# tkob-vh/umi-collapse-rs

Measured on AMD Instinct MI355X. Metric: UMI-pair Hamming comparisons/s, effective (W pairs of the positions / hot-path time; 12-bp UMIs, all-pairs adjacency + directional collapse; the n-gram partition compares walked_fraction of W, the all-pairs kernels' result bit for bit), higher is better.
Workload: dtype u32; 1 GPU; BASELINE config 2 per GPU: 1000000 reads, 12-bp UMIs, one alignment position (uniform UMIs), --data naive --algo dir -k 1 -p 0.5; standard=True, reads_per_rank=1000000, positions_per_rank=1, unique_umis_rank0=970714, pairs_W_total=471142349541, parallelism=one GPU

## Files before the change

umi_collapse_rs_amd/csrc/umihip_internal.h:

```cpp
#pragma once

#include <hip/hip_runtime_api.h>
#include <stdint.h>

namespace umihip {

struct PairTask {
    uint32_t row0;
    uint32_t row_end;
    uint32_t col0;
    uint32_t col1;
};

enum PairMode : int {
    MODE_DIRECTIONAL = 0,
    MODE_ADJACENCY = 1,
    MODE_NEIGHBOURS = 2,
    MODE_CLUSTER = 3,
};

enum Counter : int {
    CNT_EDGES = 0,
    CNT_CANDIDATES = 1,
    CNT_ERROR = 2,
// ... 157 lines not shown
    uint32_t *bin_start;
    unsigned long long *scan_state;
    SegTask *tasks;
    uint32_t task_cap;
    void *sub_rec;
    const RangeTask *ranges;
    uint32_t n_ranges;
    const SegBlock *blocks;
    uint32_t n_blocks;
    uint32_t lds_bins;
    uint32_t parts_per_pass;
    uint2 *priv_edges;
    uint8_t *priv_dist;
    uint32_t *priv_cnt;
    uint2 *priv_stat;
    uint32_t *uf_parent;
    const uint64_t *prep_keys, *prep_nmask;
    const int32_t *prep_freq;
    int32_t *prep_thr;
    uint32_t *prep_label;
    uint32_t *prep_lab;
    float prep_percentage;
    unsigned long long *prep_counters;
    int umi_len;
    int key_words;
    int full_umi_len;
    uint32_t use_ckey;
    uint32_t col_sliced;
    uint32_t local_cap;
    uint32_t probe_rest, probe_min;
    uint32_t super_cap;
    const SegSuper *supers;
    uint32_t n_supers;
};
hipError_t launch_seg_build(const SegArgs &g, void *fkey, const int32_t *freq, bool key32,
                            unsigned long long *counters, hipStream_t s);
constexpr uint32_t SEG_PRIV_CAP = 512;
int seg_pair_blocks_per_cu(bool key32, bool has_n, bool ckey);
hipError_t launch_seg_pairs(const PairArgs &a, const SegArgs &g, bool key32, float percentage,
                            uint32_t part, uint32_t n_parts, uint32_t n_blocks, hipStream_t s);
hipError_t launch_seg_edge_append(const PairArgs &a, const SegArgs &g, uint32_t n_blocks, hipStream_t s);
constexpr uint32_t SEG_LOCAL_MAX_CAP = 2048;
constexpr uint32_t SEG_LOCAL_CAP = 512;
constexpr int SEG_PROBE_MAX_REST = 6;
constexpr uint32_t SEG_PROBE_WORDS = (1u << (2 * SEG_PROBE_MAX_REST)) / 32;
constexpr uint32_t SEG_PROBE_MIN = 129;
constexpr int SEG_SUPER_MAX_REST = 8;
constexpr uint32_t SEG_SUPER_WORDS = (1u << (2 * SEG_SUPER_MAX_REST)) / 32;
constexpr int SEG_SUPER_MAX_BASES = 4;
constexpr uint32_t SEG_SUPER_MAX_CAP = 8192;
constexpr uint32_t SEG_SUPER_CAP = 5632;
constexpr uint32_t SEG_SUPER_MIN = 1024;
constexpr uint32_t SEG_SUPER_SMALL = 2048;
inline uint32_t seg_super_threads(uint32_t cap) { return cap <= SEG_SUPER_SMALL ? 256u : 1024u; }
size_t seg_super_lds_bytes(uint32_t cap);
uint32_t seg_super_blocks(uint32_t n_supers, uint32_t n_cus);
hipError_t launch_seg_super(const PairArgs &a, const SegArgs &g, float percentage, uint32_t n_blocks, hipStream_t s);
size_t seg_local_lds_bytes(uint32_t cap);
int seg_local_blocks_per_cu(bool has_n, uint32_t cap);
hipError_t launch_seg_local(const PairArgs &a, const SegArgs &g, float percentage, uint32_t n_blocks, hipStream_t s);

hipError_t launch_wide_pairs(const PairArgs &a, uint32_t n_tasks, int n_words, hipStream_t s);

hipError_t launch_edit_prep(const uint64_t *keys, const uint64_t *nmask, const int32_t *freq, const uint64_t *bucket_off,
                            uint64_t n_buckets, uint32_t n, int umi_len, float percentage, uint64_t *planes,
                            uint32_t *counts, int32_t *thr, uint32_t *label, unsigned long long *counters, hipStream_t s);
hipError_t launch_edit_pairs(const PairArgs &a, const uint32_t *counts, uint32_t n_tasks, int umi_len, hipStream_t s);
// ... 252 lines not shown
```

umi_collapse_rs_amd/csrc/umihip_pipeline.cpp:

```cpp
#include "umihip_host.hpp"

#include <algorithm>
#include <chrono>

using namespace umihip;

namespace {

template <class LaunchRound>
int run_rounds(umi_ctx *ctx, hipStream_t s, LaunchRound launch_round, int &rounds, int batch = 4)
{
    uint32_t *d_changed = ctx->d_changed();
    for (;;) {
        HIP_TRY(hipMemsetAsync(d_changed, 0, sizeof(uint32_t) * MAX_ROUNDS_PER_SYNC, s));
        for (int r = 0; r < batch; r++) HIP_TRY(launch_round(d_changed, r));
        HIP_TRY(hipMemcpyAsync(ctx->h_changed(), d_changed, sizeof(uint32_t) * batch, hipMemcpyDeviceToHost, s));
        HIP_TRY(hipStreamSynchronize(s));
        bool done = false;
        for (int r = 0; r < batch && !done; r++) {
            rounds++;
            done = ctx->h_changed()[r] == 0;
        }
        if (done) return UMI_OK;
        if (rounds > MAX_ROUNDS) return fail(UMI_ERR_HIP, "label propagation diverged");
// ... 257 lines not shown
            if ((rc = ctx->status.reserve(n)) || (rc = ctx->blocked.reserve(n))) return rc;
        if (edit && (rc = ctx->planes.reserve((size_t)n * 4))) return rc;
        d_cnt = ctx->counters.as<unsigned long long>();
        bs_fkey = ctx->fkey.p;
        return UMI_OK;
    }

    void plan_host()
    {
        scan_table_range(bucket_off, 0, n_buckets, fused_max, nullptr, ctx->table_pass);
        const bool dev_tiles = mode != MODE_CLUSTER;
        const bool seg_on = ctx->seg_index && need_pairs && !(ctx->prune && dev_tiles) && !edit;
        SegSuperOpt sup;
        sup.on = ctx->seg_super && ctx->seg_unite && ctx->seg_ckey && unions_collapse() && n_parts == 1 && ctx->two_phase == 2 &&
                 key32 && !wide() && !edit && !d_nmask;
        sup.bases = ctx->seg_super_bases;
        sup.cap = ctx->seg_super_cap;
        sup.min = ctx->seg_super_min;
        build_plan(bucket_off, n_buckets, wide() || edit ? 0x7FFFFFFFu : ctx->small_max,
                   ctx->use_bitslice && k <= BS_MAX_K && !wide() && !edit && dev_tiles,
                   plan_umi_len(), fused_max, ctx->prune && dev_tiles, ctx->bs_sorted && ctx->bs_unit == 2 && need_pairs && dev_tiles,
                   ctx->bs_tables && key32 && dev_tiles, ctx->bs_tab_min_run, seg_on ? std::max(ctx->seg_min, 1u) : 0u, k, key32, pl,
                   &ctx->table_pass, sup);
        prune = ctx->prune && dev_tiles && need_pairs && !pl.bs_buckets.empty() && !wide() && !edit;
        keep_my_share(pl.small_tasks);
        keep_my_share(pl.big_tasks);
        st.max_bucket = pl.max_bucket;
        st.n_pairs = pl.n_pairs;
    }

    size_t seg_bins_bytes() const { return (pl.seg_bins * 4 + 15) & ~(size_t)15; }
    size_t seg_zero_bytes() const
    {
        return (seg_bins_bytes() + (1 + pl.seg_chunks.size()) * sizeof(unsigned long long) + 15) & ~(size_t)15;
    }

    int upload_plan()
    {
        int rc;
        size_t off = 0;
        auto place = [&](size_t bytes) {
            const size_t at = off;
            off = (off + bytes + 63) & ~(size_t)63;
            return at;
        };
        const size_t o_ranges = place(pl.ranges.size() * sizeof(RangeTask));
        const size_t o_segs = place(pl.segs.size() * sizeof(SegDesc));
        const size_t o_chunks = place(pl.seg_chunks.size() * sizeof(SegScanChunk));
        const size_t o_blocks = place(pl.seg_blocks.size() * sizeof(SegBlock));
        const size_t o_supers = place(pl.seg_supers.size() * sizeof(SegSuper));
        const size_t o_small = place(pl.small_tasks.size() * sizeof(PairTask));
        const size_t o_big = place(pl.big_tasks.size() * sizeof(PairTask));
        const size_t total = std::max<size_t>(off, 64);
        PinnedBuf &hp = ctx->h_plan_alt[ctx->plan_flip];
        if ((rc = hp.reserve(total)) || (rc = ctx->plan_tables.reserve(total))) return rc;
        if (off) memset(hp.p, 0, off);
        if ((rc = hp.put(o_ranges, pl.ranges.data(), pl.ranges.size() * sizeof(RangeTask))) ||
            (rc = hp.put(o_segs, pl.segs.data(), pl.segs.size() * sizeof(SegDesc))) ||
            (rc = hp.put(o_chunks, pl.seg_chunks.data(), pl.seg_chunks.size() * sizeof(SegScanChunk))) ||
            (rc = hp.put(o_blocks, pl.seg_blocks.data(), pl.seg_blocks.size() * sizeof(SegBlock))) ||
            (rc = hp.put(o_supers, pl.seg_supers.data(), pl.seg_supers.size() * sizeof(SegSuper))) ||
            (rc = hp.put(o_small, pl.small_tasks.data(), pl.small_tasks.size() * sizeof(PairTask))) ||
            (rc = hp.put(o_big, pl.big_tasks.data(), pl.big_tasks.size() * sizeof(PairTask))))
            return rc;
        const PinnedBuf &prev = ctx->h_plan_alt[ctx->plan_flip ^ 1];
        const bool same = off && ctx->plan_uploaded == off && ctx->plan_uploaded_to == ctx->plan_tables.p &&
                          prev.p && prev.cap >= off && memcmp(prev.p, hp.p, off) == 0;
// ... 400 lines not shown
        const PairArgs a = pair_args(ovf_cap);
        if (pl.seg_parts) {
            const uint32_t blocks = std::max(1u, (uint32_t)std::min<uint64_t>(
                pl.seg_task_cap, ctx->seg_blocks ? ctx->seg_blocks : (uint64_t)ctx->n_cus * std::min(16u, seg_occupancy())));
            const uint32_t local_blocks = seg.local_cap && seg_local_bins ? (uint32_t)std::max<uint64_t>(1, std::min<uint64_t>(
                                                              seg_local_bins, (uint64_t)ctx->n_cus * seg_local_occupancy()))
                                                        : 0u;
            const uint32_t super_blocks = seg.super_cap ? seg_super_blocks(seg.n_supers, (uint32_t)ctx->n_cus) : 0u;
            const uint32_t super_slots = super_blocks * (seg_super_threads(seg.super_cap) / 64u);
            const size_t slots = (size_t)local_blocks + super_slots + blocks;
            if ((rc = ctx->seg_priv_edges.reserve(slots * SEG_PRIV_CAP * sizeof(uint2))) ||
                (rc = ctx->seg_priv_cnt.reserve(slots * 4)) || (rc = ctx->seg_priv_stat.reserve(slots * sizeof(uint2))) ||
                (mode == MODE_NEIGHBOURS && (rc = ctx->seg_priv_dist.reserve((size_t)blocks * SEG_PRIV_CAP))))
                return rc;
            seg.priv_edges = ctx->seg_priv_edges.as<uint2>();
            seg.priv_dist = ctx->seg_priv_dist.as<uint8_t>();
            seg.priv_cnt = ctx->seg_priv_cnt.as<uint32_t>();
            seg.uf_parent = one_sync() && ctx->seg_unite ? ctx->label.as<uint32_t>() : nullptr;
            const bool slots_to_collapse = seg.uf_parent && unions_collapse();
            seg.priv_stat = slots_to_collapse ? ctx->seg_priv_stat.as<uint2>() : nullptr;
            if ((seg.local_cap || seg.super_cap) && !seg.uf_parent)
                return fail(UMI_ERR_HIP, "internal: part-0 sub-buckets planned for the local kernel without unions");
            SegArgs super_seg = seg;
            super_seg.priv_edges += (size_t)local_blocks * SEG_PRIV_CAP;
            super_seg.priv_cnt += local_blocks;
            if (super_seg.priv_stat) super_seg.priv_stat += local_blocks;
            SegArgs pair_seg = super_seg;
            pair_seg.priv_edges += (size_t)super_slots * SEG_PRIV_CAP;
            pair_seg.priv_cnt += super_slots;
            if (pair_seg.priv_stat) pair_seg.priv_stat += super_slots;

            if (prof) HIP_TRY(hipEventRecord(ctx->ev[7], s));
            if (local_blocks) HIP_TRY(launch_seg_local(a, seg, percentage, local_blocks, s));
            if (super_blocks) HIP_TRY(launch_seg_super(a, super_seg, percentage, super_blocks, s));
            HIP_TRY(launch_seg_pairs(a, pair_seg, key32, percentage, part, n_parts, blocks, s));
            if (prof) HIP_TRY(hipEventRecord(ctx->ev[8], s));
            seg_timed = true;
            priv_blocks_for_collapse = slots_to_collapse ? (uint32_t)slots : 0u;
            if (!priv_blocks_for_collapse) HIP_TRY(launch_seg_edge_append(a, seg, blocks, s));
            st.n_pair_launches += 1;
        }
        if ((rc = enqueue_legacy_tiles(a))) return rc;
        if (edit) {
            if (prof) HIP_TRY(hipEventRecord(ctx->ev[7], s));
            HIP_TRY(launch_edit_pairs(a, ctx->planes.as<uint32_t>(), (uint32_t)pl.small_tasks.size(), umi_len, s));
            if (prof) HIP_TRY(hipEventRecord(ctx->ev[8], s));
            edit_timed = true;
            st.n_pair_launches += pl.small_tasks.empty() ? 0 : 1;
            return UMI_OK;
        }
        if (wide()) {
            HIP_TRY(launch_wide_pairs(a, (uint32_t)pl.small_tasks.size(), n_words, s));
            st.n_pair_launches += pl.small_tasks.empty() ? 0 : 1;
            return UMI_OK;
        }
        PairArgs big = a;
        big.tasks = d_big;
        HIP_TRY(launch_pairs(big, (uint32_t)pl.big_tasks.size(), true, key32, s));
        HIP_TRY(launch_pairs(a, (uint32_t)pl.small_tasks.size(), false, key32, s));
        for (auto &v : pl.bs_tasks) st.n_pair_launches += v.empty() ? 0 : 1;
        st.n_pair_launches += pl.tab_rows.empty() ? 0 : 2;
        st.n_pair_launches += (pl.small_tasks.empty() ? 0 : 1) + (pl.big_tasks.empty() ? 0 : 1);
        return UMI_OK;
    }

    int note_pair_counters()
    {
// ... 387 lines not shown
```

umi_collapse_rs_amd/csrc/umihip_seg.hip:

```cpp
#include <hip/hip_runtime.h>

#include "umihip_internal.h"
#include "umihip_device.h"

namespace umihip {

namespace {

constexpr int SCAN_THREADS = 256;
constexpr int SCAN_PER_THREAD = SEG_SCAN_CHUNK / SCAN_THREADS;

__device__ __forceinline__ bool probe_part(const SegArgs &g, uint32_t nb)
{
    return g.probe_rest != 0u && g.umi_len - (int)nb <= (int)g.probe_rest;
}
__device__ __forceinline__ bool local_bin(const SegArgs &g, uint32_t part, uint32_t c) { return part == 0 && c <= g.local_cap; }
__device__ __forceinline__ bool super_taken(const SegArgs &g, uint32_t n) { return n >= 2u && n <= g.super_cap; }
__device__ __forceinline__ uint32_t super_bases(const SegArgs &g, uint32_t seg) { return g.super_cap ? g.segs[seg].sup_g : 0u; }

constexpr unsigned long long SCAN_HAVE = 1ull << 63, SCAN_PREFIX = 1ull << 31;
__device__ __forceinline__ unsigned long long scan_pack(uint32_t e, uint32_t t) { return ((unsigned long long)e << 32) | t; }
__global__ __launch_bounds__(SCAN_THREADS) void seg_scan_kernel(SegArgs g, unsigned long long *counters)
{
    __shared__ uint2 wsum[SCAN_THREADS / 64];
    __shared__ uint32_t my_chunk;
    __shared__ uint2 prefix;
    unsigned long long *ticket = g.scan_state, *status = g.scan_state + 1;
    if (threadIdx.x == 0) my_chunk = (uint32_t)atomicAdd(ticket, 1ull);
    __syncthreads();
    const uint32_t ci = my_chunk;
    const SegScanChunk ch = g.chunks[ci];
    uint32_t c[SCAN_PER_THREAD];
    uint2 mine = make_uint2(0u, 0u);
    const uint32_t b_first = threadIdx.x * SCAN_PER_THREAD;
#pragma unroll
    for (int q = 0; q < SCAN_PER_THREAD; q++) {
        const uint32_t b = b_first + q;
        c[q] = b < ch.nbins ? g.bin_cnt[ch.bin0 + b] : 0u;
        mine.x += c[q];
    }
    uint32_t no_tasks = 0;
    const uint32_t sg = ch.part == 0 ? super_bases(g, ch.seg) : 0u;
    if (sg) {
        static_assert(SCAN_PER_THREAD == 1 || SCAN_PER_THREAD == 4, "a super-bin is whole threads' bins");
        __shared__ uint32_t tcnt[SCAN_THREADS];
        tcnt[threadIdx.x] = mine.x;
        __syncthreads();
        const uint32_t nthr = (1u << (2 * sg)) / SCAN_PER_THREAD, t0 = threadIdx.x & ~(nthr - 1u);
        uint32_t n_super = 0;
        for (uint32_t i = 0; i < nthr; i++) n_super += tcnt[t0 + i];
        if (super_taken(g, n_super)) no_tasks = (1u << SCAN_PER_THREAD) - 1u;
    } else {
#pragma unroll
        for (int q = 0; q < SCAN_PER_THREAD; q++)
            if (local_bin(g, ch.part, c[q])) no_tasks |= 1u << q;
    }
#pragma unroll
    for (int q = 0; q < SCAN_PER_THREAD; q++) mine.y += (no_tasks >> q) & 1u ? 0u : seg_tasks_of_bin(c[q]);
    uint2 incl = mine;
    for (int d = 1; d < 64; d <<= 1) {
        const uint32_t ux = __shfl_up(incl.x, d), uy = __shfl_up(incl.y, d);
        if ((int)(threadIdx.x & 63) >= d) {
            incl.x += ux;
            incl.y += uy;
        }
    }
    if ((threadIdx.x & 63) == 63) wsum[threadIdx.x >> 6] = incl;
    __syncthreads();
    if (threadIdx.x < 64) {
        uint2 tot = make_uint2(0u, 0u);
        for (int w = 0; w < SCAN_THREADS / 64; w++) {
            tot.x += wsum[w].x;
            tot.y += wsum[w].y;
        }
        const int lane = threadIdx.x;
        if (lane == 0)
            __hip_atomic_store(&status[ci], SCAN_HAVE | (ci == 0 ? SCAN_PREFIX : 0ull) | scan_pack(tot.x, tot.y),
                               __ATOMIC_RELEASE, __HIP_MEMORY_SCOPE_AGENT);
        uint2 before = make_uint2(0u, 0u);
        int64_t j0 = (int64_t)ci - 1;
        while (j0 >= 0) {
            const int64_t j = j0 - lane;
            unsigned long long st = SCAN_HAVE | SCAN_PREFIX;
            if (j >= 0)
// ... 323 lines not shown
            "v_addc_co_u32_e64 %0, vcc, %0, %0, %11\n\t"
            "v_addc_co_u32_e64 %0, vcc, %0, %0, %12"
            : "+v"(h), "=&s"(s0), "=&s"(s1), "=&s"(s2), "=&s"(s3), "=&v"(t0), "=&v"(t1), "=&v"(t2), "=&v"(t3),
              "=&s"(p0), "=&s"(p1), "=&s"(p2), "=&s"(p3)
            : "v"(x), "v"(ky), "s"(lim2), "n"(J), "n"(J - 1), "n"(J - 2), "n"(J - 3)
            : "vcc");
        return h;
    }
#pragma unroll
    for (int j = J; j > J - 4; j--) h = h + h + (within_k(x ^ readlane_key(ky, j), k) ? 1u : 0u);
    return h;
}
template <bool CK, int J> __device__ __forceinline__ uint32_t four_columns(uint32_t h, uint64_t x, uint64_t ky, int k, uint32_t)
{
#pragma unroll
    for (int j = J; j > J - 4; j--) h = h + h + (within_k(x ^ readlane_key(ky, j), k) ? 1u : 0u);
    return h;
}
template <bool CK, int BASE, typename KeyT>
__device__ __forceinline__ uint32_t columns32(KeyT x, KeyT ky, int k, uint32_t lim2)
{
    uint32_t h = 0;
    h = four_columns<CK, BASE + 31>(h, x, ky, k, lim2);
    h = four_columns<CK, BASE + 27>(h, x, ky, k, lim2);
    h = four_columns<CK, BASE + 23>(h, x, ky, k, lim2);
    h = four_columns<CK, BASE + 19>(h, x, ky, k, lim2);
    h = four_columns<CK, BASE + 15>(h, x, ky, k, lim2);
    h = four_columns<CK, BASE + 11>(h, x, ky, k, lim2);
    h = four_columns<CK, BASE + 7>(h, x, ky, k, lim2);
    h = four_columns<CK, BASE + 3>(h, x, ky, k, lim2);
    return h;
}

template <int K, int NB> __device__ __forceinline__ unsigned long long columns64_sliced(uint32_t x, uint32_t ky)
{
    uint32_t cl[K + 1], ch[K + 1];
#pragma unroll
    for (int l = 0; l <= K; l++) cl[l] = ch[l] = 0u;
#pragma unroll
    for (int b = 0; b < NB; b++) {
        const unsigned long long p0 = __ballot((ky & (1u << (3 * b))) != 0u), p1 = __ballot((ky & (2u << (3 * b))) != 0u);
        const uint32_t r0 = (uint32_t)((int32_t)(x << (31 - 3 * b)) >> 31), r1 = (uint32_t)((int32_t)(x << (30 - 3 * b)) >> 31);
        const uint32_t dl = BITOP3((uint32_t)p0 ^ r0, (uint32_t)p1, r1, TT_A | (TT_B ^ TT_C));
        const uint32_t dh = BITOP3((uint32_t)(p0 >> 32) ^ r0, (uint32_t)(p1 >> 32), r1, TT_A | (TT_B ^ TT_C));
#pragma unroll
        for (int l = K; l >= 1; l--) {
            cl[l] = BITOP3(cl[l], cl[l - 1], dl, TT_A | (TT_B & TT_C));
            ch[l] = BITOP3(ch[l], ch[l - 1], dh, TT_A | (TT_B & TT_C));
        }
        cl[0] |= dl;
        ch[0] |= dh;
    }
    return ~(((unsigned long long)ch[K] << 32) | cl[K]);
}
template <int K> __device__ __forceinline__ unsigned long long columns64_sliced_nb(uint32_t x, uint32_t ky, int nb)
{
    switch (nb) {
    case 1: return columns64_sliced<K, 1>(x, ky);
    case 2: return columns64_sliced<K, 2>(x, ky);
    case 3: return columns64_sliced<K, 3>(x, ky);
    case 4: return columns64_sliced<K, 4>(x, ky);
    case 5: return columns64_sliced<K, 5>(x, ky);
    case 6: return columns64_sliced<K, 6>(x, ky);
    case 7: return columns64_sliced<K, 7>(x, ky);
    case 8: return columns64_sliced<K, 8>(x, ky);
    case 9: return columns64_sliced<K, 9>(x, ky);
    default: return columns64_sliced<K, 10>(x, ky);
    }
}
__device__ __forceinline__ unsigned long long columns64_sliced_k(uint32_t x, uint32_t ky, int k, int nb)
{
    switch (k) {
    case 0: return columns64_sliced_nb<0>(x, ky, nb);
    case 1: return columns64_sliced_nb<1>(x, ky, nb);
    case 2: return columns64_sliced_nb<2>(x, ky, nb);
    default: return columns64_sliced_nb<3>(x, ky, nb);
    }
}
__device__ __forceinline__ unsigned long long columns64_sliced_k(uint64_t, uint64_t, int, int) { return 0ull; }

template <int ILP>
__device__ __forceinline__ void uf_union_multi(uint32_t *parent, uint32_t (&u)[ILP], uint32_t (&v)[ILP], bool (&act)[ILP])
{
    uint32_t pu[ILP], pv[ILP];
    uint32_t seen[ILP];
#pragma unroll
    for (int s = 0; s < ILP; s++) seen[s] = act[s] ? atomicCAS(&parent[v[s]], v[s], u[s]) : 0u;
#pragma unroll
    for (int s = 0; s < ILP; s++) act[s] = act[s] && seen[s] != v[s] && seen[s] != u[s];
#pragma unroll
    for (int s = 0; s < ILP; s++) {
        pu[s] = act[s] ? ld_parent(&parent[u[s]]) : 0u;
        pv[s] = seen[s];
    }
    for (;;) {
        bool cas[ILP], any = false;
#pragma unroll
        for (int s = 0; s < ILP; s++) {
            act[s] = act[s] && pu[s] != pv[s];
            if (act[s] && pu[s] < pv[s]) {
                uint32_t t = u[s]; u[s] = v[s]; v[s] = t;
                t = pu[s]; pu[s] = pv[s]; pv[s] = t;
            }
            cas[s] = act[s] && u[s] == pu[s];
            any = any || act[s];
        }
        if (!any) break;
        uint32_t r[ILP];
#pragma unroll
        for (int s = 0; s < ILP; s++)
            r[s] = !act[s] ? 0u : cas[s] ? atomicCAS(&parent[u[s]], u[s], pv[s]) : ld_parent(&parent[pu[s]]);
#pragma unroll
// ... 7 lines not shown
                pu[s] = r[s];
            }
        }
    }
}

template <typename KeyT, bool HAS_N, bool CK, int W = 1>
__global__ __launch_bounds__(64) void seg_pair_kernel(PairArgs a, SegArgs g, float percentage,
                                                      uint32_t part, uint32_t n_parts)
{
    using Rec = typename SegRecOf<KeyT>::type;
    constexpr int ILP = 1;
    constexpr uint32_t DRAIN_AT = 64 * ILP;
    constexpr uint32_t HITQ = DRAIN_AT + 64;
    __shared__ EdgeStage stage;
    __shared__ uint2 hitq[HITQ];
    const int lane = threadIdx.x;
    const Rec *__restrict__ sub = (const Rec *)g.sub_rec;
    const uint4 *__restrict__ task_words = (const uint4 *)g.tasks;
    const bool with_dist = a.mode == MODE_NEIGHBOURS;
    if (lane == 0) {
        stage.count = 0;
        stage.candidates = 0;
    }
    __syncthreads();
    const uint32_t n_tasks = (uint32_t)min((unsigned long long)g.task_cap, a.counters[CNT_SEG_TASKS]);
    unsigned int n_cand = 0, n_direct = 0;
    const uint32_t lim2 = (uint32_t)__builtin_amdgcn_readfirstlane(2 * a.k);
    KeyT dup_mask[SEG_MAX_PARTS - 1];
#pragma unroll
    for (int j = 0; j < SEG_MAX_PARTS - 1; j++) dup_mask[j] = KeyT(0);
    uint32_t have_seg = SEG_NONE, have_part = 0;
    int ck_bases = 0;
    uint32_t sup_mask = 0, sup_bins = 0, sup_bin0 = 0;
    const bool sliced = a.k <= 3 && g.col_sliced != 0;
    uint32_t nq = 0;

    auto drain = [&]() {
        __builtin_amdgcn_wave_barrier();
        for (uint32_t q0 = 0; q0 < nq; q0 += 64 * ILP) {
            Rec ra[ILP], cb[ILP];
            bool live[ILP];
#pragma unroll
            for (int s = 0; s < ILP; s++) {
                const uint32_t q = q0 + (uint32_t)s * 64u + (uint32_t)lane;
                live[s] = q < nq;
                const uint2 h = live[s] ? hitq[q] : make_uint2(0u, 0u);
                ra[s] = sub[live[s] ? h.x : 0u];
                cb[s] = sub[live[s] ? h.y : 0u];
            }
            uint32_t uu[ILP], uv[ILP];
            bool unite[ILP];
#pragma unroll
            for (int s = 0; s < ILP; s++) {
                unite[s] = false;
                uu[s] = uv[s] = 0;
                if (!live[s]) continue;
                const KeyT z = ra[s].key ^ cb[s].key;
                bool ok = true;
#pragma unroll
                for (int p = 0; p < SEG_MAX_PARTS - 1; p++)
                    ok = ok && (dup_mask[p] == KeyT(0) || (z & dup_mask[p]) != KeyT(0));
                if (!ok) continue;
                if (sup_bins && ((uint32_t)z & sup_mask) == 0u) {
                    const uint32_t b = sup_bin0 + ((uint32_t)ra[s].key & sup_mask);
                    if (super_taken(g, g.bin_start[b + sup_bins] - g.bin_start[b])) continue;
                }
// ... 72 lines not shown
    uint4 tw = t < n_tasks ? task_words[t] : none;
    uint4 tw1 = t + stride < n_tasks && t + stride > t ? task_words[t + stride] : none;
    KeyT x, ky;
    task_keys(tw, t < n_tasks, x, ky);
    while (t < n_tasks) {
        const uint32_t t1 = t + stride, t2 = t1 + stride;
        const bool has1 = t1 < n_tasks && t1 > t, has2 = has1 && t2 < n_tasks && t2 > t1;
        const uint4 tw2 = has2 ? task_words[t2] : none;
        KeyT x1, ky1;
        task_keys(tw1, has1, x1, ky1);
        const uint32_t row0 = __builtin_amdgcn_readfirstlane(tw.x);
        const uint32_t end = __builtin_amdgcn_readfirstlane(tw.y);
        const uint32_t col0 = __builtin_amdgcn_readfirstlane(tw.z);
        const uint32_t where = __builtin_amdgcn_readfirstlane(tw.w);
        const uint32_t seg = where & 0xFFFFFFu, my_part = (where >> 24) & 15u;
        const uint32_t col1 = (uint32_t)min((unsigned long long)end, (unsigned long long)col0 + (64ull << (where >> 28)));
        const bool mine = !(n_parts > 1 && (((end ^ (end >> 7)) * 0x9E3779B1u) >> 8) % n_parts != part);
        if (mine) {
            const uint32_t n_rows = min(64u, end - row0);
            const uint32_t r = row0 + (uint32_t)lane;
            if (seg != have_seg || my_part != have_part) {
                if (nq) drain();
                const SegDesc *__restrict__ sd = g.segs + seg;
#pragma unroll
                for (int j = 0; j < SEG_MAX_PARTS - 1; j++)
                    dup_mask[j] = (uint32_t)j < my_part ? (KeyT)sd->mask[j] : KeyT(0);
                have_seg = seg;
                have_part = my_part;
                ck_bases = __builtin_amdgcn_readfirstlane(g.umi_len - (int)sd->nb[my_part]);
                const uint32_t sg = my_part != 0 ? super_bases(g, seg) : 0u;
                sup_mask = sg ? ((1u << (2 * (sd->nb[0] - sg))) - 1u) << (2 * sg) : 0u;
                sup_bins = sg ? 1u << (2 * sg) : 0u;
                sup_bin0 = sd->bin_off[0];
            }
            for (uint32_t c0 = col0; c0 < col1; c0 += 64) {
                const uint32_t cn_pos = c0 + 64u + (uint32_t)lane;
                KeyT kn = pad_col<KeyT>();
                if (c0 + 64u < col1 && cn_pos < end) kn = loop_key<CK>(sub[cn_pos]);
                const uint32_t nc = min(64u, end - c0);
                unsigned long long h;
                if (CK && sliced) {
                    h = columns64_sliced_k(x, ky, a.k, ck_bases);
                } else {
                    uint32_t hlo = 0, hhi = 0;
                    hlo = columns32<CK, 0>(x, ky, a.k, lim2);
                    if (nc > 32) hhi = columns32<CK, 32>(x, ky, a.k, lim2);
                    h = ((unsigned long long)hhi << 32) | hlo;
                }
                const int j_min = lane + 1 - (int)(c0 - row0);
                if (nc < 64) h &= (1ull << nc) - 1ull;
                if (j_min > 0) h = j_min >= 64 ? 0ull : h & ~((1ull << j_min) - 1ull);
                if ((uint32_t)lane >= n_rows) h = 0ull;
                while (__any(h != 0ull)) {
                    const unsigned long long bal = __ballot(h != 0ull);
                    if (h) {
                        const int j = __builtin_ctzll(h);
                        h &= h - 1ull;
                        hitq[nq + (uint32_t)__builtin_popcountll(bal & ((1ull << lane) - 1ull))] =
                            make_uint2(r, c0 + (uint32_t)j);
                    }
                    nq += (uint32_t)__builtin_popcountll(bal);
                    if (nq >= DRAIN_AT) drain();
                }
                ky = kn;
            }
        }
        if (!has1) break;
        t = t1;
        tw = tw1;
        tw1 = tw2;
        x = x1;
        ky = ky1;
    }
    if (nq) drain();
    {
// ... 257 lines not shown
                            h &= h - 1ull;
                            hit = r | ((c0 + (uint32_t)j) << 16);
                        }
                        push(has, hit);
                    }
                }
            }
        }
        if (nq) drain();
        for (uint32_t p = lane; p < c; p += 64) {
            uint32_t q = lds_ld(&par[p]);
            for (;;) {
                const uint32_t up = lds_ld(&par[q]);
                if (up == q) break;
                q = up;
            }
            ck[p] = q;
            fr[p] = 0xFFFFFFFFu;
        }
        __syncthreads();
        for (uint32_t p = lane; p < c; p += 64) atomicMin(&fr[ck[p]], ix[p]);
        __syncthreads();
        for (uint32_t p = lane; p < c; p += 64) g.uf_parent[ix[p]] = fr[ck[p]];
        __syncthreads();
    }
    if (lane == 0) g.priv_cnt[blockIdx.x] = min(n_out, SEG_PRIV_CAP);
    for (int off = 32; off > 0; off >>= 1) n_cand += __shfl_down(n_cand, off);
    for (int off = 32; off > 0; off >>= 1) n_direct += __shfl_down(n_direct, off);
    if (lane == 0) g.priv_stat[blockIdx.x] = make_uint2(n_cand, n_direct);
}

constexpr int SUPER_RPT = 8;

template <bool CLUSTER, int NT>
__global__ __launch_bounds__(NT) void seg_super_kernel(PairArgs a, SegArgs g, float percentage)
{
    extern __shared__ uint32_t lds[];
    constexpr int NW = NT / 64;
    constexpr int WPT = (int)SEG_SUPER_WORDS / NT;
    static_assert(WPT * NT == (int)SEG_SUPER_WORDS && WPT >= 1, "whole words per thread");
    const uint32_t cap = g.super_cap;
    uint32_t *sc = lds, *ix = lds + cap, *fr = lds + 2 * cap, *par = lds + 3 * cap;
    uint32_t *bm = lds + 4 * cap, *pre = bm + SEG_SUPER_WORDS;
    __shared__ uint32_t wsum[NW];
    const uint32_t tid = threadIdx.x, wave = tid >> 6;
    const int lane = (int)(tid & 63u);
    const SegRec32 *__restrict__ sub = (const SegRec32 *)g.sub_rec;
    unsigned int n_cand = 0, n_direct = 0;
    const size_t my_slot = (size_t)blockIdx.x * NW + wave;
    uint32_t n_out = 0;
    uint2 *__restrict__ slot = g.priv_edges + my_slot * SEG_PRIV_CAP;
    auto emit = [&](bool has, uint32_t u, uint32_t v) {
        const unsigned long long bal = __ballot(has);
        if (!bal) return;
        const uint32_t cnt = (uint32_t)__builtin_popcountll(bal);
        const uint32_t pos = n_out + (uint32_t)__builtin_popcountll(bal & ((1ull << lane) - 1ull));
        unsigned long long base = 0;
        if (n_out + cnt > SEG_PRIV_CAP) {
            const uint32_t first_over = max(n_out, SEG_PRIV_CAP);
            const int leader = __builtin_ctzll(bal);
            if (lane == leader) base = atomicAdd(&a.counters[CNT_EDGES], (unsigned long long)(n_out + cnt - first_over));
            base = __shfl(base, leader);
            base -= first_over;
        }
        if (has) {
            if (pos < SEG_PRIV_CAP) slot[pos] = make_uint2(u, v);
            else if (base + pos < a.edge_cap) a.edges[base + pos] = make_uint2(u, v);
        }
        n_out += cnt;
    };
    auto decide = [&](bool has, uint32_t pa, uint32_t pb) {
        const uint32_t ia = ix[pa], ib = ix[pb];
        const int32_t fa = (int32_t)fr[pa], fb = (int32_t)fr[pb];
        const bool sw = ib < ia;
        const uint32_t gi = sw ? ib : ia, gj = sw ? ia : ib;
        const int32_t fi = sw ? fb : fa, fj = sw ? fa : fb;
        if (has) n_cand++;
        const bool fwd = has && (CLUSTER || fj <= threshold_of(percentage, fi));
        const bool bwd = has && (CLUSTER || fi <= threshold_of(percentage, fj));
        if (fwd && bwd) {
            n_direct++;
            lds_union_halving(par, min(pa, pb), max(pa, pb));
        }
        emit(fwd != bwd, fwd ? gi : gj, fwd ? gj : gi);
    };

    for (uint32_t u = blockIdx.x; u < g.n_supers; u += gridDim.x) {
        const SegSuper su = g.supers[u];
        const uint32_t start = __builtin_amdgcn_readfirstlane(g.bin_start[su.bin0]);
        const uint32_t c = __builtin_amdgcn_readfirstlane(g.bin_start[su.bin0 + (1u << (2 * su.g))]) - start;
        if (!super_taken(g, c)) continue;
        const uint32_t lo_bits = 2u * su.g, hi_shift = 2u * su.nb, rest = su.rest;
        const uint32_t lo_mask = (1u << lo_bits) - 1u, code_mask = (1u << (2u * rest)) - 1u;
        for (uint32_t w = tid; w < SEG_SUPER_WORDS; w += NT) bm[w] = 0u;
        uint32_t rc[SUPER_RPT], ri[SUPER_RPT], rf[SUPER_RPT], rq[SUPER_RPT];
#pragma unroll
        for (int r = 0; r < SUPER_RPT; r++) {
            const uint32_t p = tid + (uint32_t)r * NT;
            rc[r] = ri[r] = rf[r] = rq[r] = 0u;
            if (p < c) {
                const SegRec32 rec = sub[start + p];
                rc[r] = ((rec.key & lo_mask) | ((rec.key >> hi_shift) << lo_bits)) & code_mask;
                ri[r] = rec.idx;
                rf[r] = (uint32_t)rec.freq;
            }
        }
        __syncthreads();
        bool twice = false;
#pragma unroll
        for (int r = 0; r < SUPER_RPT; r++)
            if (tid + (uint32_t)r * NT < c) {
                const uint32_t bit = 1u << (rc[r] & 31u);
                twice = twice || (atomicOr(&bm[rc[r] >> 5], bit) & bit) != 0u;
            }
        const bool dup = __syncthreads_or(twice ? 1 : 0) != 0;
        if (!dup) {
            {
                uint32_t n_w[WPT], mine = 0;
#pragma unroll
                for (int i = 0; i < WPT; i++) mine += n_w[i] = (uint32_t)__builtin_popcount(bm[tid * WPT + i]);
                uint32_t incl = mine;
                for (int d = 1; d < 64; d <<= 1) {
                    const uint32_t up = __shfl_up(incl, d);
                    if (lane >= d) incl += up;
                }
                if (lane == 63) wsum[wave] = incl;
                __syncthreads();
                uint32_t before = incl - mine;
                for (uint32_t w = 0; w < wave; w++) before += wsum[w];
#pragma unroll
                for (int i = 0; i < WPT; i++) {
                    pre[tid * WPT + i] = before;
                    before += n_w[i];
                }
            }
            __syncthreads();
            auto rank_of = [&](uint32_t s) {
                return pre[s >> 5] + (uint32_t)__builtin_popcount(bm[s >> 5] & ((1u << (s & 31u)) - 1u));
            };
#pragma unroll
            for (int r = 0; r < SUPER_RPT; r++)
                if (tid + (uint32_t)r * NT < c) {
                    const uint32_t q = rank_of(rc[r]);
                    rq[r] = q;
                    sc[q] = rc[r];
                    ix[q] = ri[r];
                    fr[q] = rf[r];
                    par[q] = q;
                }
            __syncthreads();
#pragma unroll
            for (int r = 0; r < SUPER_RPT; r++) {
                if ((uint32_t)r * NT >= c) break;
                const uint32_t s = rc[r];
                uint32_t m = 0;
#pragma unroll
                for (int bb = 0; bb < SEG_SUPER_MAX_REST; bb++) {
#pragma unroll
                    for (int d = 1; d <= 3; d++) {
                        const uint32_t t = s ^ ((uint32_t)d << (2 * bb));
                        const uint32_t there = (bm[t >> 5] >> (t & 31u)) & 1u;
                        if ((uint32_t)bb < rest && t > s) m |= there << (3 * bb + d - 1);
                    }
                }
                if (tid + (uint32_t)r * NT >= c) m = 0u;
                while (__any(m != 0u)) {
                    const bool has = m != 0u;
                    uint32_t pb = 0;
                    if (has) {
                        const int j = __builtin_ctz(m), bb = j / 3;
                        m &= m - 1u;
                        pb = rank_of(s ^ ((uint32_t)(j - 3 * bb + 1) << (2 * bb)));
                    }
                    decide(has, has ? rq[r] : 0u, pb);
                }
            }
        } else {
#pragma unroll
            for (int r = 0; r < SUPER_RPT; r++) {
                const uint32_t p = tid + (uint32_t)r * NT;
                if (p < c) {
                    sc[p] = rc[r];
                    ix[p] = ri[r];
                    fr[p] = rf[r];
                    par[p] = p;
                }
            }
            __syncthreads();
#pragma unroll
            for (int r = 0; r < SUPER_RPT; r++) {
                if ((uint32_t)r * NT >= c) break;
                const uint32_t p = tid + (uint32_t)r * NT, p_first = p - (uint32_t)lane;
                const uint32_t s = rc[r];
                const uint32_t n_it = c > p_first + 1u ? c - 1u - p_first : 0u;
                for (uint32_t i = 1; i <= n_it; i++) {
                    const uint32_t q = p + i;
                    const uint32_t z = s ^ (q < c ? sc[q] : 0u);
                    const bool hit = p < c && q < c && __builtin_popcount((z | (z >> 1)) & 0x55555555u) <= 1;
                    if (__any(hit)) decide(hit, hit ? p : 0u, hit ? q : 0u);
                }
            }
        }
        __syncthreads();
        for (;;) {
            bool moved = false;
            for (uint32_t p = tid; p < c; p += NT) {
                const uint32_t q = lds_ld(&par[p]), up = lds_ld(&par[q]);
                if (up != q) {
                    __hip_atomic_store(&par[p], up, __ATOMIC_RELAXED, __HIP_MEMORY_SCOPE_WORKGROUP);
                    moved = true;
                }
            }
            if (!__syncthreads_or(moved ? 1 : 0)) break;
        }
        for (uint32_t p = tid; p < c; p += NT) sc[p] = lds_ld(&par[p]);
        __syncthreads();
        for (uint32_t p = tid; p < c; p += NT) fr[p] = 0xFFFFFFFFu;
        __syncthreads();
        for (uint32_t p = tid; p < c; p += NT) atomicMin(&fr[sc[p]], ix[p]);
        __syncthreads();
        for (uint32_t p = tid; p < c; p += NT) g.uf_parent[ix[p]] = fr[sc[p]];
        __syncthreads();
    }
    if (lane == 0) g.priv_cnt[my_slot] = min(n_out, SEG_PRIV_CAP);
    for (int off = 32; off > 0; off >>= 1) n_cand += __shfl_down(n_cand, off);
    for (int off = 32; off > 0; off >>= 1) n_direct += __shfl_down(n_direct, off);
    if (lane == 0) g.priv_stat[my_slot] = make_uint2(n_cand, n_direct);
}

__global__ __launch_bounds__(1024) void seg_edge_scan_kernel(uint32_t *priv_cnt, uint32_t n_blocks,
                                                             unsigned long long *counters)
{
    __shared__ uint32_t wsum[16];
    __shared__ uint32_t carry;
    if (threadIdx.x == 0) carry = 0;
    __syncthreads();
    const unsigned long long base = counters[CNT_EDGES];
    for (uint32_t b0 = 0; b0 < n_blocks; b0 += 1024) {
        const uint32_t i = b0 + threadIdx.x;
        const uint32_t v = i < n_blocks ? priv_cnt[i] : 0u;
        uint32_t incl = v;
        for (int d = 1; d < 64; d <<= 1) {
            const uint32_t up = __shfl_up(incl, d);
            if ((int)(threadIdx.x & 63) >= d) incl += up;
        }
        if ((threadIdx.x & 63) == 63) wsum[threadIdx.x >> 6] = incl;
        __syncthreads();
        uint32_t off = carry;
        for (uint32_t w = 0; w < (threadIdx.x >> 6); w++) off += wsum[w];
        if (i < n_blocks) priv_cnt[i] = (uint32_t)min(base + off + incl - v, 0xFFFFFFFFull);
        __syncthreads();
        if (threadIdx.x == 1023) carry = off + incl;
        __syncthreads();
    }
    if (threadIdx.x == 0) counters[CNT_EDGES] = base + carry;
// ... 158 lines not shown
```

Before: 1856000 billion UMI-pair comparisons/s.

## Skip super-bin columns in sliced pair tiles when every super-bucket is handled by the super kernel

The scan kernel now sets a per-segment flag word when a super-bucket's count exceeds super_cap. When no such overflow is flagged, the sliced pair kernel switches from excluding super bins to a column-tile mask, so it keeps only the columns that differ on the super bases and skips pairs the super kernel already handled. This cuts redundant Hamming tests in the generic pair kernel at the cost of an extra flag read and more template instantiations. Dev-only per-phase timing stamps for the super kernel are also added behind UMIHIP_DEV.

New measurement: 1888000 billion UMI-pair comparisons/s (median of 6 runs). 1.8% higher.

```diff
diff --git a/umi_collapse_rs_amd/csrc/umihip_internal.h b/umi_collapse_rs_amd/csrc/umihip_internal.h
--- a/umi_collapse_rs_amd/csrc/umihip_internal.h
+++ b/umi_collapse_rs_amd/csrc/umihip_internal.h
@@ -213,7 +213,12 @@
     uint32_t super_cap;
     const SegSuper *supers;
     uint32_t n_supers;
-};
+#ifdef UMIHIP_DEV
+    unsigned long long *super_stamps;
+#endif
+};
+constexpr int SEG_SUPER_PHASES = 8;
+UMIHIP_HD inline uint32_t seg_scan_flag_word(uint32_t n_chunks, uint32_t seg) { return 1u + n_chunks + seg; }
 hipError_t launch_seg_build(const SegArgs &g, void *fkey, const int32_t *freq, bool key32,
                             unsigned long long *counters, hipStream_t s);
 constexpr uint32_t SEG_PRIV_CAP = 512;
diff --git a/umi_collapse_rs_amd/csrc/umihip_pipeline.cpp b/umi_collapse_rs_amd/csrc/umihip_pipeline.cpp
--- a/umi_collapse_rs_amd/csrc/umihip_pipeline.cpp
+++ b/umi_collapse_rs_amd/csrc/umihip_pipeline.cpp
@@ -313,7 +313,7 @@
     size_t seg_bins_bytes() const { return (pl.seg_bins * 4 + 15) & ~(size_t)15; }
     size_t seg_zero_bytes() const
     {
-        return (seg_bins_bytes() + (1 + pl.seg_chunks.size()) * sizeof(unsigned long long) + 15) & ~(size_t)15;
+        return (seg_bins_bytes() + (1 + pl.seg_chunks.size() + pl.segs.size()) * sizeof(unsigned long long) + 15) & ~(size_t)15;
     }
 
     int upload_plan()
@@ -780,7 +780,43 @@
 
             if (prof) HIP_TRY(hipEventRecord(ctx->ev[7], s));
             if (local_blocks) HIP_TRY(launch_seg_local(a, seg, percentage, local_blocks, s));
+#ifdef UMIHIP_DEV
+            const char *phase_file = super_blocks ? getenv("UMIHIP_SUPER_PHASES") : nullptr;
+            if (phase_file && *phase_file) {
+                const size_t n_stamps = (size_t)super_blocks * SEG_SUPER_PHASES;
+                HIP_TRY(hipMalloc((void **)&super_seg.super_stamps, n_stamps * sizeof(unsigned long long)));
+                HIP_TRY(hipMemsetAsync(super_seg.super_stamps, 0, n_stamps * sizeof(unsigned long long), s));
+            }
+#endif
             if (super_blocks) HIP_TRY(launch_seg_super(a, super_seg, percentage, super_blocks, s));
+#ifdef UMIHIP_DEV
+            if (super_seg.super_stamps) {
+                std::vector<unsigned long long> ticks((size_t)super_blocks * SEG_SUPER_PHASES);
+                const hipError_t e = hipMemcpyAsync(ticks.data(), super_seg.super_stamps, ticks.size() * sizeof(unsigned long long),
+                                                    hipMemcpyDeviceToHost, s);
+                const hipError_t e2 = e == hipSuccess ? hipStreamSynchronize(s) : e;
+                (void)hipFree(super_seg.super_stamps);
+                HIP_TRY(e2);
+                if (FILE *f = fopen(phase_file, "a")) {
+                    static const char *const names[SEG_SUPER_PHASES] = {"records in", "map built", "ranks and placement",
+                        "bit tests (wave 0)", "hit rounds", "pointer jumping", "atomicMin", "label stores"};
+                    fprintf(f, "seg_super_kernel: %u blocks, us per block (100 MHz clock): phase, mean, max\n", super_blocks);
+                    double sum_mean = 0;
+                    for (int i = 0; i < SEG_SUPER_PHASES; i++) {
+                        unsigned long long tot = 0, mx = 0;
+                        for (uint32_t b = 0; b < super_blocks; b++) {
+                            const unsigned long long t = ticks[(size_t)b * SEG_SUPER_PHASES + i];
+                            tot += t;
+                            mx = std::max(mx, t);
+                        }
+                        sum_mean += (double)tot / super_blocks / 100.0;
+                        fprintf(f, "  %-22s %8.2f %8.2f\n", names[i], (double)tot / super_blocks / 100.0, (double)mx / 100.0);
+                    }
+                    fprintf(f, "  %-22s %8.2f\n", "all phases", sum_mean);
+                    fclose(f);
+                }
+            }
+#endif
             HIP_TRY(launch_seg_pairs(a, pair_seg, key32, percentage, part, n_parts, blocks, s));
             if (prof) HIP_TRY(hipEventRecord(ctx->ev[8], s));
             seg_timed = true;
diff --git a/umi_collapse_rs_amd/csrc/umihip_seg.hip b/umi_collapse_rs_amd/csrc/umihip_seg.hip
--- a/umi_collapse_rs_amd/csrc/umihip_seg.hip
+++ b/umi_collapse_rs_amd/csrc/umihip_seg.hip
@@ -50,6 +50,7 @@
         uint32_t n_super = 0;
         for (uint32_t i = 0; i < nthr; i++) n_super += tcnt[t0 + i];
         if (super_taken(g, n_super)) no_tasks = (1u << SCAN_PER_THREAD) - 1u;
+        if (n_super > g.super_cap && threadIdx.x == t0) g.scan_state[seg_scan_flag_word(g.n_chunks, ch.seg)] = 1ull;
     } else {
 #pragma unroll
         for (int q = 0; q < SCAN_PER_THREAD; q++)
@@ -439,9 +440,10 @@
     return h;
 }
 
-template <int K, int NB> __device__ __forceinline__ unsigned long long columns64_sliced(uint32_t x, uint32_t ky)
-{
-    uint32_t cl[K + 1], ch[K + 1];
+template <int K, int NB, bool SUP = false>
+__device__ __forceinline__ unsigned long long columns64_sliced(uint32_t x, uint32_t ky, uint32_t sup_bases = 0)
+{
+    uint32_t cl[K + 1], ch[K + 1], sl = 0, sh = 0;
 #pragma unroll
     for (int l = 0; l <= K; l++) cl[l] = ch[l] = 0u;
 #pragma unroll
@@ -457,11 +459,29 @@
         }
         cl[0] |= dl;
         ch[0] |= dh;
-    }
+        if (SUP && (sup_bases >> b) & 1u) {
+            sl |= dl;
+            sh |= dh;
+        }
+    }
+    if (SUP) return (((unsigned long long)(sh & ~ch[K]) << 32) | (sl & ~cl[K]));
     return ~(((unsigned long long)ch[K] << 32) | cl[K]);
 }
-template <int K> __device__ __forceinline__ unsigned long long columns64_sliced_nb(uint32_t x, uint32_t ky, int nb)
-{
+template <int K> __device__ __forceinline__ unsigned long long columns64_sliced_nb(uint32_t x, uint32_t ky, int nb, uint32_t sup_bases)
+{
+    if (K == 1 && sup_bases)
+        switch (nb) {
+        case 1: return columns64_sliced<1, 1, true>(x, ky, sup_bases);
+        case 2: return columns64_sliced<1, 2, true>(x, ky, sup_bases);
+        case 3: return columns64_sliced<1, 3, true>(x, ky, sup_bases);
+        case 4: return columns64_sliced<1, 4, true>(x, ky, sup_bases);
+        case 5: return columns64_sliced<1, 5, true>(x, ky, sup_bases);
+        case 6: return columns64_sliced<1, 6, true>(x, ky, sup_bases);
+        case 7: return columns64_sliced<1, 7, true>(x, ky, sup_bases);
+        case 8: return columns64_sliced<1, 8, true>(x, ky, sup_bases);
+        case 9: return columns64_sliced<1, 9, true>(x, ky, sup_bases);
+        default: return columns64_sliced<1, 10, true>(x, ky, sup_bases);
+        }
     switch (nb) {
     case 1: return columns64_sliced<K, 1>(x, ky);
     case 2: return columns64_sliced<K, 2>(x, ky);
@@ -475,16 +495,16 @@
     default: return columns64_sliced<K, 10>(x, ky);
     }
 }
-__device__ __forceinline__ unsigned long long columns64_sliced_k(uint32_t x, uint32_t ky, int k, int nb)
+__device__ __forceinline__ unsigned long long columns64_sliced_k(uint32_t x, uint32_t ky, int k, int nb, uint32_t sup_bases = 0)
 {
     switch (k) {
-    case 0: return columns64_sliced_nb<0>(x, ky, nb);
-    case 1: return columns64_sliced_nb<1>(x, ky, nb);
-    case 2: return columns64_sliced_nb<2>(x, ky, nb);
-    default: return columns64_sliced_nb<3>(x, ky, nb);
-    }
-}
-__device__ __forceinline__ unsigned long long columns64_sliced_k(uint64_t, uint64_t, int, int) { return 0ull; }
+    case 0: return columns64_sliced_nb<0>(x, ky, nb, 0u);
+    case 1: return columns64_sliced_nb<1>(x, ky, nb, sup_bases);
+    case 2: return columns64_sliced_nb<2>(x, ky, nb, 0u);
+    default: return columns64_sliced_nb<3>(x, ky, nb, 0u);
+    }
+}
+__device__ __forceinline__ unsigned long long columns64_sliced_k(uint64_t, uint64_t, int, int, uint32_t = 0) { return 0ull; }
 
 template <int ILP>
 __device__ __forceinline__ void uf_union_multi(uint32_t *parent, uint32_t (&u)[ILP], uint32_t (&v)[ILP], bool (&act)[ILP])
@@ -558,7 +578,7 @@
     for (int j = 0; j < SEG_MAX_PARTS - 1; j++) dup_mask[j] = KeyT(0);
     uint32_t have_seg = SEG_NONE, have_part = 0;
     int ck_bases = 0;
-    uint32_t sup_mask = 0, sup_bins = 0, sup_bin0 = 0;
+    uint32_t sup_mask = 0, sup_bins = 0, sup_bin0 = 0, sup_tile = 0;
     const bool sliced = a.k <= 3 && g.col_sliced != 0;
     uint32_t nq = 0;
 
@@ -697,6 +717,11 @@
                 sup_mask = sg ? ((1u << (2 * (sd->nb[0] - sg))) - 1u) << (2 * sg) : 0u;
                 sup_bins = sg ? 1u << (2 * sg) : 0u;
                 sup_bin0 = sd->bin_off[0];
+                sup_tile = 0u;
+                if (CK && sliced && sg && sg < sd->nb[0] && __builtin_amdgcn_readfirstlane((uint32_t)g.scan_state[seg_scan_flag_word(g.n_chunks, seg)]) == 0u) {
+                    sup_tile = ((1u << sd->nb[0]) - 1u) & ~((1u << sg) - 1u);
+                    sup_bins = 0u;
+                }
             }
             for (uint32_t c0 = col0; c0 < col1; c0 += 64) {
                 const uint32_t cn_pos = c0 + 64u + (uint32_t)lane;
@@ -705,7 +730,7 @@
                 const uint32_t nc = min(64u, end - c0);
                 unsigned long long h;
                 if (CK && sliced) {
-                    h = columns64_sliced_k(x, ky, a.k, ck_bases);
+                    h = columns64_sliced_k(x, ky, a.k, ck_bases, sup_tile);
                 } else {
                     uint32_t hlo = 0, hhi = 0;
                     hlo = columns32<CK, 0>(x, ky, a.k, lim2);
@@ -1029,6 +1054,17 @@
 
 constexpr int SUPER_RPT = 8;
 
+#ifdef UMIHIP_DEV
+__device__ __forceinline__ unsigned long long super_clock()
+{
+    unsigned long long t;
+    __builtin_amdgcn_sched_barrier(0);
+    asm volatile("s_waitcnt vmcnt(0) lgkmcnt(0)\n\ts_memrealtime %0\n\ts_waitcnt lgkmcnt(0)" : "=s"(t) : : "memory");
+    __builtin_amdgcn_sched_barrier(0);
+    return t;
+}
+#endif
+
 template <bool CLUSTER, int NT>
 __global__ __launch_bounds__(NT) void seg_super_kernel(PairArgs a, SegArgs g, float percentage)
 {
@@ -1066,6 +1102,17 @@
         }
         n_out += cnt;
     };
+#ifdef UMIHIP_DEV
+    unsigned long long t_prev = g.super_stamps ? super_clock() : 0ull;
+    auto stamp = [&](int i) {
+        if (!g.super_stamps) return;
+        const unsigned long long now = super_clock();
+        if (tid == 0) g.super_stamps[(size_t)blockIdx.x * SEG_SUPER_PHASES + i] += now - t_prev;
+        t_prev = now;
+    };
+#else
+    auto stamp = [](int) {};
+#endif
     auto decide = [&](bool has, uint32_t pa, uint32_t pb) {
         const uint32_t ia = ix[pa], ib = ix[pb];
         const int32_t fa = (int32_t)fr[pa], fb = (int32_t)fr[pb];
@@ -1103,6 +1150,7 @@
             }
         }
         __syncthreads();
+        stamp(0);
         bool twice = false;
 #pragma unroll
         for (int r = 0; r < SUPER_RPT; r++)
@@ -1111,6 +1159,7 @@
                 twice = twice || (atomicOr(&bm[rc[r] >> 5], bit) & bit) != 0u;
             }
         const bool dup = __syncthreads_or(twice ? 1 : 0) != 0;
+        stamp(1);
         if (!dup) {
             {
                 uint32_t n_w[WPT], mine = 0;
@@ -1146,6 +1195,7 @@
                     par[q] = q;
                 }
             __syncthreads();
+            stamp(2);
 #pragma unroll
             for (int r = 0; r < SUPER_RPT; r++) {
                 if ((uint32_t)r * NT >= c) break;
@@ -1161,6 +1211,7 @@
                     }
                 }
                 if (tid + (uint32_t)r * NT >= c) m = 0u;
+                stamp(3);
                 while (__any(m != 0u)) {
                     const bool has = m != 0u;
                     uint32_t pb = 0;
@@ -1171,6 +1222,7 @@
                     }
                     decide(has, has ? rq[r] : 0u, pb);
                 }
+                stamp(4);
             }
         } else {
 #pragma unroll
@@ -1184,6 +1236,7 @@
                 }
             }
             __syncthreads();
+            stamp(2);
 #pragma unroll
             for (int r = 0; r < SUPER_RPT; r++) {
                 if ((uint32_t)r * NT >= c) break;
@@ -1199,6 +1252,7 @@
             }
         }
         __syncthreads();
+        stamp(4);
         for (;;) {
             bool moved = false;
             for (uint32_t p = tid; p < c; p += NT) {
@@ -1210,14 +1264,17 @@
             }
             if (!__syncthreads_or(moved ? 1 : 0)) break;
         }
+        stamp(5);
         for (uint32_t p = tid; p < c; p += NT) sc[p] = lds_ld(&par[p]);
         __syncthreads();
         for (uint32_t p = tid; p < c; p += NT) fr[p] = 0xFFFFFFFFu;
         __syncthreads();
         for (uint32_t p = tid; p < c; p += NT) atomicMin(&fr[sc[p]], ix[p]);
         __syncthreads();
+        stamp(6);
         for (uint32_t p = tid; p < c; p += NT) g.uf_parent[ix[p]] = fr[sc[p]];
         __syncthreads();
+        stamp(7);
     }
     if (lane == 0) g.priv_cnt[my_slot] = min(n_out, SEG_PRIV_CAP);
     for (int off = 32; off > 0; off >>= 1) n_cand += __shfl_down(n_cand, off);
```
